# GadGadGad/Convolutional-KAN-for-Image-Classification

Hardware: AMD Instinct MI355X
Metric: images/sec fwd+bwd KAN-VGG11 3x32x32 bs=256/GPU (higher is better)
Workload: dtype f32

## Files before the change

### convolutional-kan-for-image-classification_amd/_lib.py

```python
from __future__ import annotations

import ctypes as C
import os
from typing import Optional

_HERE = os.path.dirname(os.path.abspath(__file__))
LIB_PATH = os.environ.get("KANCONV_LIB") or os.path.join(_HERE, "libkanconv.so")

KAN_MAX_PLANES = 16
KAN_MAX_TABLE = 32
KAN_FP_WORDS = 192
BASIS_BSPLINE, BASIS_RBF, BASIS_CHEBY, BASIS_POLY, BASIS_FOURIER, BASIS_RELU, BASIS_GRAM = 0, 1, 2, 3, 4, 5, 6
ACT_NONE, ACT_IDENTITY, ACT_GELU, ACT_SILU, ACT_RELU, ACT_TANH, ACT_SIGMOID, ACT_GELU_TANH = -1, 0, 1, 2, 3, 4, 5, 6
ORDER_QUAD_FWD, ORDER_ROWBLK8_FWD, ORDER_QUAD_BWD_DATA, ORDER_FWD_WEIGHT_SIDE = 1, 2, 4, 8


class KanGeom(C.Structure):
    _fields_ = [(n, C.c_int) for n in ("B", "C", "H", "W", "O", "Ho", "Wo", "kh", "kw", "sh", "sw", "ph", "pw", "dh", "dw", "groups")] + \
               [("x_bstride", C.c_longlong), ("y_bstride", C.c_longlong)]


class KanBasis(C.Structure):
    _fields_ = [("kind", C.c_int), ("n_basis", C.c_int), ("order", C.c_int), ("act", C.c_int),
                ("p0", C.c_float), ("p1", C.c_float), ("table", C.c_float * KAN_MAX_TABLE), ("chan_table", C.c_void_p)]


class KanPlan(C.Structure):
    _fields_ = [(n, C.c_int) for n in ("P", "K", "IPC", "KC", "Kpad", "Opad", "fwd_splits", "bwd_data_splits", "bwd_weight_splits",
                                          "fwd_target", "bwd_data_target", "bwd_weight_target", "x_pm_wanted", "dz_pm_wanted", "bwd_weight_expanded", "row_blocks", "e_pm_wanted", "fwd_expanded", "fwd_halo", "bwd_weight_halo",
                                          "fwd_band", "bwd_weight_band")] + \
               [(n, C.c_longlong) for n in ("packed_weight_bytes", "bwd_data_weight_bytes", "fwd_slab_elems", "bwd_data_slab_elems",
                                            "bwd_weight_slab_elems", "e_pm_elems")]


class KanNormRoute(C.Structure):
    _fields_ = [(n, C.c_int) for n in ("kernel", "G", "EPL", "PPI", "NT", "pool", "lds", "held", "blocks", "strided")]


NORM_GENERIC, NORM_REGS = 0, 1
NORM_POOL_NONE, NORM_POOL_2X2, NORM_POOL_K = 0, 1, 2


class KanWavGeom(C.Structure):
    _fields_ = [(n, C.c_int) for n in ("B", "C", "H", "W", "O", "Ho", "Wo", "kh", "kw", "sh", "sw", "ph", "pw", "dh", "dw", "wavelet")] + \
               [("x_bstride", C.c_longlong), ("u_bstride", C.c_longlong)]


# ... 113 lines not shown
```

### convolutional-kan-for-image-classification_amd/csrc/kan_common.h

```cpp
#pragma once
#include <hip/hip_runtime.h>
#include <cstdint>
#include <type_traits>
#include "kanconv.h"
#include "kan_device.h"
#include "kan_internal.h"

typedef float f32x16 __attribute__((ext_vector_type(16)));
#define MFMA32(a, b, c) __builtin_amdgcn_mfma_f32_32x32x2f32((a), (b), (c), 0, 0, 0)
#define LDS_READ4(r0, r1, r2, r3, addrA, addrB, o0, o1, o2, o3)                                                        \
    asm volatile("ds_read_b32 %0, %4 offset:%6\n\tds_read_b32 %1, %4 offset:%7\n\tds_read_b32 %2, %5 offset:%8\n\tds_read_b32 %3, %5 offset:%9" \
                 : "=&v"(r0), "=&v"(r1), "=&v"(r2), "=&v"(r3) : "v"(addrA), "v"(addrB), "n"(o0), "n"(o1), "n"(o2), "n"(o3) : "memory")
#define LDS_WAIT4(r0, r1, r2, r3, N) asm volatile("s_waitcnt lgkmcnt(" #N ")" : "+v"(r0), "+v"(r1), "+v"(r2), "+v"(r3) :: "memory")
__device__ __forceinline__ unsigned lds_addr(const float* p) { return (unsigned)(size_t)(__attribute__((address_space(3))) const float*)p; }
#define KAN_MFMA_STEP(NK, addrA, LDA, addrB, LDB)                                                                                   \
    do {                                                                                                                           \
        float fa_[2][2], fb_[2][2];                                                                                                \
        LDS_READ4(fa_[0][0], fa_[0][1], fb_[0][0], fb_[0][1], addrA, addrB, 0, 32 * 4, 0, 32 * 4);                                 \
        _Pragma("unroll") for (int kk = 0; kk < (NK); ++kk) {                                                                       \
            const int c_ = kk & 1, n_ = c_ ^ 1;                                                                                    \
            if (kk + 1 < (NK)) {                                                                                                   \
                LDS_READ4(fa_[n_][0], fa_[n_][1], fb_[n_][0], fb_[n_][1], addrA, addrB, (2 * (kk + 1)) * (LDA) * 4,                \
                          (2 * (kk + 1)) * (LDA) * 4 + 128, (2 * (kk + 1)) * (LDB) * 4, (2 * (kk + 1)) * (LDB) * 4 + 128);         \
                LDS_WAIT4(fa_[c_][0], fa_[c_][1], fb_[c_][0], fb_[c_][1], 4);                                                      \
            } else {                                                                                                               \
                LDS_WAIT4(fa_[c_][0], fa_[c_][1], fb_[c_][0], fb_[c_][1], 0);                                                      \
            }                                                                                                                      \
            acc[0][0] = MFMA32(fa_[c_][0], fb_[c_][0], acc[0][0]);                                                                 \
            acc[0][1] = MFMA32(fa_[c_][0], fb_[c_][1], acc[0][1]);                                                                 \
            acc[1][0] = MFMA32(fa_[c_][1], fb_[c_][0], acc[1][0]);                                                                 \
            acc[1][1] = MFMA32(fa_[c_][1], fb_[c_][1], acc[1][1]);                                                                 \
        }                                                                                                                          \
    } while (0)

#define KAN_MFMA_STEP_LIVE(NK, addrA, LDA, addrB, LDB, l0a, l0b, l1a, l1b)                                                          \
    do {                                                                                                                           \
        float fa_[2][2], fb_[2][2];                                                                                                \
        LDS_READ4(fa_[0][0], fa_[0][1], fb_[0][0], fb_[0][1], addrA, addrB, 0, 32 * 4, 0, 32 * 4);                                 \
        _Pragma("unroll") for (int kk = 0; kk < (NK); ++kk) {                                                                       \
            const int c_ = kk & 1, n_ = c_ ^ 1;                                                                                    \
            if (kk + 1 < (NK)) {                                                                                                   \
                LDS_READ4(fa_[n_][0], fa_[n_][1], fb_[n_][0], fb_[n_][1], addrA, addrB, (2 * (kk + 1)) * (LDA) * 4,                \
                          (2 * (kk + 1)) * (LDA) * 4 + 128, (2 * (kk + 1)) * (LDB) * 4, (2 * (kk + 1)) * (LDB) * 4 + 128);         \
                LDS_WAIT4(fa_[c_][0], fa_[c_][1], fb_[c_][0], fb_[c_][1], 4);                                                      \
            } else {                                                                                                               \
                LDS_WAIT4(fa_[c_][0], fa_[c_][1], fb_[c_][0], fb_[c_][1], 0);                                                      \
            }                                                                                                                      \
            if (kk < (NK) / 2 ? (l0a) : (l0b)) {                                                                                   \
                acc[0][0] = MFMA32(fa_[c_][0], fb_[c_][0], acc[0][0]);                                                             \
                acc[1][0] = MFMA32(fa_[c_][1], fb_[c_][0], acc[1][0]);                                                             \
            }                                                                                                                      \
            if (kk < (NK) / 2 ? (l1a) : (l1b)) {                                                                                   \
                acc[0][1] = MFMA32(fa_[c_][0], fb_[c_][1], acc[0][1]);                                                             \
                acc[1][1] = MFMA32(fa_[c_][1], fb_[c_][1], acc[1][1]);                                                             \
            }                                                                                                                      \
        }                                                                                                                          \
    } while (0)

namespace {

struct FastDiv { unsigned m; int s; };
__host__ __device__ inline FastDiv make_fastdiv(int d) {
    FastDiv f; f.s = 0;
    while ((1ll << f.s) < d) ++f.s;
    f.m = (unsigned)((((1ull << f.s) - (unsigned long long)d) << 32) / (unsigned long long)d + 1ull);
    return f;
}
__device__ __forceinline__ int fastdiv(int a, FastDiv f) {
    if (f.s == 0) return a;
    const unsigned t = __umulhi((unsigned)a, f.m);
    return (int)((t + (((unsigned)a - t) >> 1)) >> (f.s - 1));
}

template <int G>
__device__ __forceinline__ float group_sum(float v) {
#pragma unroll
    for (int off = G / 2; off >= 1; off >>= 1) v += __shfl_xor(v, off, 64);
    return v;
}
template <int G>
__device__ __forceinline__ double group_sum(double v) {
#pragma unroll
    for (int off = G / 2; off >= 1; off >>= 1) v += __shfl_xor(v, off, 64);
    return v;
}

struct DevGeom {
    int B, C, H, W, O, Ho, Wo, kh, kw, sh, sw, ph, pw, dh, dw;
    int howo_shift, wo_shift;
    int pix_major;
// ... 309 lines not shown
```

### convolutional-kan-for-image-classification_amd/csrc/kan_internal.h

```cpp
#pragma once
#include <type_traits>
#include "kanconv.h"

int kan_fail_msg(const char* fmt, const char* a);
int kan_raise_lds_limit(const void* kernel, int bytes);

enum : int {
    FAST_GENERIC = 0,
    FAST_BSPLINE_SILU = 1,
    FAST_BSPLINE_GELU = 2,
    FAST_RBF8 = 3,
    FAST_CHEBY5 = 4,
    FAST_CHEBY4 = 5,
    FAST_POLY4 = 6,
    FAST_POLY3 = 7,
    FAST_RBF5 = 8,
    FAST_RELU8 = 9,
    FAST_GRAM4 = 10,
    FAST_POLY1 = 11,
    FAST_LAST = 11
};
enum : unsigned {
    ON_TAP_MAJOR = 1u << 0,
    ON_BIG_TILES = 1u << 1,
// ... 75 lines not shown
    unsigned short bw_ph_rt0[KAN_BAND_MAX_PHASES + 1];
    unsigned char ph_a[KAN_BAND_MAX_PHASES], ph_b[KAN_BAND_MAX_PHASES];
    short ph_tap0[KAN_BAND_MAX_PHASES + 1];
    unsigned short tap_shift[KAN_BAND_MAX_TAPS];
    unsigned short tap_rt[KAN_BAND_MAX_TAPS];
    short tap_step[KAN_BAND_MAX_TAPS], tap_nt[KAN_BAND_MAX_TAPS];
} KanBandCfg;

void kan_band_cfg(const KanGeom* g, const KanBasis* b, int fast, KanBandCfg* cfg);
int kan_band_bwd_weight_launch(const float* dz, const float* x, const float* xn, float* dwp, const KanGeom* g, const KanBasis* b,
                               const KanBandCfg* cfg, int splits, long long slab_elems, void* stream);
int kan_band_fwd_launch(const float* x, const float* xn, const float* wp, float* z, const KanGeom* g, const KanBasis* b,
                        const KanBandCfg* cfg, int splits, long long slab_elems, void* stream);

constexpr int DW_T = 9;
constexpr int DW_MAX_TP = 96;

enum class Route { TAP_MAJOR, DW, BAND, HALO, EXPANDED };

struct FwdCfg { int TO, TP, tiles_o, tiles_p, chunks, splits, slots; };
struct BdCfg { int CH, tiles_c, tiles_p, n_ob, Opad32, chunks, splits; };
struct BwCfg { int TR, TO, tiles_r, tiles_o, chunks, splits, slots; };
struct BwHaloCfg { int R, nimg, spb, n_bands, tiles_r, tiles_o, splits, bands_per_split; };

struct ConvPlan {
    KanPlan pub;
    int fast;
    Route fwd, bwd_data, bwd_weight;
    bool pm_fwd, pm_bwd_data, pm_bwd_weight;
    bool rowblk_bwd_data;
    bool quad_fwd;
    bool quad_bd;
    bool rowblk8_fwd;
    bool fwd_wq;
    bool pmdma_xcd, pm_lpt, pm_xcd;
    FwdCfg fc;
    BdCfg bd;
    BwCfg bw;
    BwHaloCfg bwh;
    KanBandCfg band;
};
int plan_conv(const KanGeom* g, const KanBasis* b, ConvPlan* cp);

int live_taps_out(const KanGeom* g, int hw);
int live_taps_in(const KanGeom* g, int hw);
int live_positions_for_tap(const KanGeom* g, int tap);
int balance_tiles(const int* weight, int n, unsigned short* idx);
```

### convolutional-kan-for-image-classification_amd/csrc/kan_plan.hip

```cpp
#include <hip/hip_runtime.h>
#include <cstdio>
#include <cstdlib>
#include <cstring>
#include "kanconv.h"
#include "kan_device.h"
#include "kan_common.h"
#include "kan_internal.h"

namespace {

int fail(const char* msg) { return kan_fail_msg("%s", msg); }

int check(const KanGeom* g, const KanBasis* b) {
    if (!g || !b) return fail("null geometry/basis");
    if (g->groups < 0 || g->groups > 65535) return fail("groups out of range");
    if (g->B <= 0 || g->C <= 0 || g->O <= 0 || g->H <= 0 || g->W <= 0 || g->Ho <= 0 || g->Wo <= 0) return fail("non-positive dimension");
    if (g->kh <= 0 || g->kw <= 0 || g->sh <= 0 || g->sw <= 0 || g->dh <= 0 || g->dw <= 0 || g->ph < 0 || g->pw < 0) return fail("bad conv parameters");
    if (g->kh > 255 || g->kw > 255 || g->C > 65535) return fail("kernel size / channel count out of supported range");
    if ((g->H + 2 * g->ph - g->dh * (g->kh - 1) - 1) / g->sh + 1 != g->Ho || (g->W + 2 * g->pw - g->dw * (g->kw - 1) - 1) / g->sw + 1 != g->Wo)
        return fail("Ho/Wo inconsistent with H/W, kernel, stride, padding, dilation");
    if ((long long)g->B * g->Ho * g->Wo >= (1ll << 31) || (long long)g->B * g->H * g->W >= (1ll << 31)) return fail("pixel count exceeds int32");
    if ((long long)g->B * g->x_bstride * 4 >= (1ll << 31) || (long long)g->B * g->y_bstride * 4 >= (1ll << 31))
        return fail("activation tensors must be smaller than 2 GiB (32-bit buffer offsets)");
    if (g->x_bstride < (long long)ngroups(g) * g->C * g->H * g->W || g->y_bstride < (long long)ngroups(g) * g->O * g->Ho * g->Wo)
// ... 101 lines not shown
    if (g->kh != 3 || g->kw != 3 || g->sh != 1 || g->sw != 1 || g->dh != 1 || g->dw != 1 || g->ph != 1 || g->pw != 1) return false;
    if ((g->C & 1) || g->O % 128 != 0) return false;
    if (pm_fwd) return false;
    const int W = g->W, H = g->H;
    return (W == 32 && H % 4 == 0) || (W == 16 && H % 8 == 0) || (W == 8 && H == 8) || (W == 4 && H == 4);
}
bool band_fwd(const KanGeom* g, const KanBasis* b, int f, bool dw, bool pm_fwd, bool halo, KanBandCfg* out) {
    if (tuning_off("KAN_BAND") || !fast_has(f, ON_BAND_FWD)) return false;
    if (b->kind == KAN_BASIS_POLY && b->order == 0) return false;
    if (dw || pm_fwd || halo) return false;
    if (!(g->C <= 3 || round_up(g->O, 64) % 128 != 0 || (g->kh * g->kw >= 4 && g->C % 2 == 0 && !tuning_off("KAN_BAND_WIDE")))) return false;
    kan_band_cfg(g, b, f, out);
    return out->ok != 0;
}
FwdCfg fwd_cfg(const KanGeom* g, const KanPlan& pl, bool big, bool pm_fwd, bool halo) {
    FwdCfg c;
    c.TO = (big && !pm_fwd) ? 256 : (pl.Opad % 128 == 0) ? 128 : 64;
    c.slots = c.TO == 256 ? 512 : 1024;
    c.TP = 128;
    c.tiles_o = pl.Opad / c.TO;
    c.tiles_p = ceil_div((long long)g->B * g->Ho * g->Wo, c.TP);
    c.chunks = pl.Kpad / pl.KC;
    c.splits = pick_splits((long long)c.tiles_o * c.tiles_p * ngroups(g), c.chunks, 8, 4.0 * g->B * g->O * g->Ho * g->Wo * ngroups(g), c.slots);
    if (halo) {
        const int n_pairs = g->C / 2, pps = ceil_div(n_pairs, c.splits < n_pairs ? c.splits : n_pairs);
        c.splits = ceil_div(n_pairs, pps);
    }
    return c;
}
bool rowblk_bwd_data(const KanGeom* g, int f, bool pm_bwd_data) {
    return !tuning_off("KAN_BD_ROWBLK") && fast_has(f, ON_ROWBLK_BWD_DATA) && !pm_bwd_data && g->H == 4 && g->W == 4 && g->Ho == 4 && g->Wo == 4 &&
           g->kh == 3 && g->kw == 3 && g->sh == 1 && g->sw == 1 && g->ph == 1 && g->pw == 1 && g->dh == 1 && g->dw == 1 && g->B % 8 == 0 && g->O % 16 == 0;
}
struct LiveClass { long long tiles; int live_steps; };

int pick_target_steps(const LiveClass* cls, int ncls, int min_steps, double slab_bytes, int* max_splits, long long SLOTS = 1024) {
    int hi = 1;
    for (int i = 0; i < ncls; ++i) if (cls[i].live_steps > hi) hi = cls[i].live_steps;
    int best = hi; double best_cost = -1; int best_ms = 1;
    for (int t = min_steps < hi ? min_steps : hi; t <= hi; ++t) {
        long long wgs = 0; int ms = 1;
        for (int i = 0; i < ncls; ++i) {
            const int sp = cls[i].live_steps > 0 ? ceil_div(cls[i].live_steps, t) : 1;
            wgs += cls[i].tiles * sp;
            if (sp > ms) ms = sp;
        }
        const long long rounds = (wgs + SLOTS - 1) / SLOTS;
        const double cost = (double)(rounds * (t + 6)) + ms * slab_cost_steps(slab_bytes);
        if (best_cost < 0 || cost < best_cost) { best_cost = cost; best = t; best_ms = ms; }
    }
    *max_splits = best_ms;
    return best;
}
BdCfg bd_cfg(const KanGeom* g, const KanPlan& pl) {
    BdCfg c;
    c.CH = 64 / pl.P;
    c.tiles_c = ceil_div(g->C, 2 * c.CH);
    c.tiles_p = ceil_div((long long)g->B * g->H * g->W, 128);
    c.n_ob = ceil_div(g->O, 16);
    c.Opad32 = round_up(g->O, 32);
    c.chunks = g->kh * g->kw * c.n_ob;
    c.splits = pick_splits((long long)c.tiles_c * c.tiles_p * ngroups(g), c.chunks, 8, 4.0 * g->B * g->C * g->H * g->W * ngroups(g));
    return c;
}
bool pmdma_bwd_weight(const KanGeom* g, const KanBasis* b, int f, bool want_pm_bw) {
    if (tuning_off("KAN_PMDMA") || !fast_has(f, ON_EXPANDED)) return false;
// ... 98 lines not shown
        order[j] = v;
    }
    for (int r = 0; r < n; ++r) {
        const int depth = r / 8, k = r % 8, bin = (depth & 1) ? 7 - k : k;
        int slot = depth * 8 + bin;
        if (slot >= n) slot = r;
        idx[slot] = (unsigned short)order[r];
    }
    bool seen[PERM_MAX] = {false};
    for (int i = 0; i < n; ++i) { if (idx[i] >= n || seen[idx[i]]) return 0; seen[idx[i]] = true; }
    return n;
}

int plan_conv(const KanGeom* g, const KanBasis* b, ConvPlan* cp) {
    if (int rc = check(g, b)) return rc;
    ConvPlan& c = *cp;
    KanPlan* pl = &c.pub;
    const int T = g->kh * g->kw, G = ngroups(g), f = fast_variant(b);
    c.fast = f;
    const bool pm_shape = pmdma_fwd_shape(g, f);
    c.pm_fwd = want_pix_major(g, b, PM_FWD, pm_shape);
    c.pm_bwd_data = want_pix_major(g, b, PM_BWD_DATA, false);
    const bool want_pm_bw = want_pix_major(g, b, PM_BWD_WEIGHT, false);
    const bool dw = dw_direct(g, b);
    const bool halo = halo_fwd(g, b, f, c.pm_fwd);
    c.band.ok = c.band.bw_ok = 0;
    const bool band = band_fwd(g, b, f, dw, c.pm_fwd, halo, &c.band);
    const bool pmdma_fwd = pm_shape && c.pm_fwd;
    const bool pmdma_bw = pmdma_bwd_weight(g, b, f, want_pm_bw);
    const bool halo_bw = halo_bwd_weight(g, f, pmdma_bw);
    c.pm_bwd_weight = want_pm_bw && !halo_bw;
    const bool band_bw = band && c.band.bw_ok && !want_pm_bw && !tuning_off("KAN_BAND_BW");
    c.rowblk_bwd_data = rowblk_bwd_data(g, f, c.pm_bwd_data);
    c.pmdma_xcd = tuning_on("KAN_PMDMA_XCD");
    c.pm_lpt = !tuning_off("KAN_PM_LPT");
    c.pm_xcd = !tuning_off("KAN_PM_XCD");
    c.fwd = dw ? Route::DW : band ? Route::BAND : halo ? Route::HALO : pmdma_fwd ? Route::EXPANDED : Route::TAP_MAJOR;
    c.bwd_data = dw ? Route::DW : Route::TAP_MAJOR;
    c.bwd_weight = dw ? Route::DW : band_bw ? Route::BAND : halo_bw ? Route::HALO : pmdma_bw ? Route::EXPANDED : Route::TAP_MAJOR;
    pl->P = b->n_basis + (b->act != KAN_ACT_NONE);
    pl->K = g->C * T * pl->P;
    {
        int i18 = 18 / pl->P, i16 = 16 / pl->P;
        if (i18 > 4) i18 = 4;
        if (i16 > 4) i16 = 4;
        const bool use18 = (long long)i18 * pl->P * 16 > (long long)i16 * pl->P * 18;
        pl->KC = use18 ? 18 : 16;
        pl->IPC = use18 ? i18 : i16;
        if (pl->P >= 10 && pl->P <= 12) { pl->KC = 12; pl->IPC = 1; }
        if (halo) { pl->KC = 2 * pl->P; pl->IPC = 2; }
    }
    pl->Kpad = ceil_div(g->C * T, pl->IPC) * pl->KC;
    if (band) { pl->KC = c.band.NPLE; pl->IPC = c.band.NG; pl->Kpad = c.band.n_steps * c.band.NPLE; }
    pl->Opad = round_up(g->O, 64);
    pl->packed_weight_bytes = (long long)G * pl->Kpad * pl->Opad * 4;
    c.bd = bd_cfg(g, *pl);
    pl->bwd_data_weight_bytes = (long long)G * T * c.bd.Opad32 * c.bd.tiles_c * 128 * 4;
    pl->fwd_slab_elems = (long long)g->B * g->y_bstride;
    pl->bwd_data_slab_elems = (long long)g->B * g->x_bstride;
    pl->bwd_weight_slab_elems = (long long)G * pl->K * pl->Opad;
    const bool big = big_tiles(f, *pl);
    c.fc = fwd_cfg(g, *pl, big, c.pm_fwd, halo);
    c.bw = bw_cfg(g, *pl, big, c.pm_bwd_weight);
    if (halo_bw) c.bwh = bw_halo_cfg(g, *pl);
    pl->fwd_splits = band ? c.band.fwd_splits : c.fc.splits;
    pl->bwd_data_splits = c.bd.splits;
// ... 50 lines not shown
```

### convolutional-kan-for-image-classification_amd/csrc/kanconv.hip

```cpp
#include <hip/hip_runtime.h>
#include <cstdio>
#include <cstdlib>
#include <cstring>
#include <cmath>
#include <cstdint>
#include <mutex>
#include <type_traits>
#include <vector>
#include "kanconv.h"
#include "kan_device.h"

#include "kan_common.h"
#include "kan_internal.h"

namespace {


thread_local char g_err[512] = "";
int fail(const char* fmt, const char* a = "") {
    snprintf(g_err, sizeof(g_err), fmt, a);
    return -1;
}
}
int kan_fail_msg(const char* fmt, const char* a) { return fail(fmt, a); }
// ... 2731 lines not shown
    if (iod) {
        const IodLaunch l = iod_launch(g, pl);
        hipLaunchKernelGGL(k_pack_iod, dim3(l.blocks), dim3(256), 0, st, w_basis, wp, q, l.o_tiles, l.n_tiles, iod_vec(w_basis, wp, g, b));
    } else {
        hipLaunchKernelGGL(k_pack, grid, dim3(256), 0, st, w_base, w_basis, wp, q, nb_base, wp_gs, tiles_x, tiles_y, fp, fp_cur);
    }
    if (wd && cp.bwd_data == Route::DW) {
        if (hipMemcpyAsync(wd, wp, (size_t)pl.packed_weight_bytes, hipMemcpyDeviceToDevice, st) != hipSuccess) return fail("memcpy failed");
    } else if (wd) {
        const BdCfg& c = cp.bd;
        const int bx = c.tiles_c * 4, by = c.Opad32 / 32 * G;
        const long long nt = (long long)bx * by;
        const long long capd = fp ? 128 : 1024;
        dim3 gd((unsigned)(nt < capd ? nt : capd), 1, T);
        hipLaunchKernelGGL(k_pack_bwd_data, gd, dim3(256), 0, st, (const float*)wp, wd, q, c.CH, c.tiles_c, c.Opad32, wp_gs, bx, by, fp, fp_cur);
    }
    return launch_ok("pack");
}

int kan_pack_weights(const float* w_base, const float* w_basis, float* wp, float* wd, const KanGeom* g, const KanBasis* b, void* stream) {
    return pack_weights_impl(w_base, w_basis, wp, wd, g, b, nullptr, 0, stream);
}

int kan_pack_weights_iod(const float* coeffs, float* wp, float* wd, const KanGeom* g, const KanBasis* b, void* stream) {
    if (int rc = iod_scope(g, b)) return rc;
    return pack_weights_impl(nullptr, coeffs, wp, wd, g, b, nullptr, 0, stream, true);
}

int kan_tile_orders(const KanGeom* g, const KanBasis* b) {
    ConvPlan cp;
    if (plan_conv(g, b, &cp)) return 0;
    const bool halo = cp.fwd == Route::HALO;
    return (halo && cp.quad_fwd ? KAN_ORDER_QUAD_FWD : 0) | (halo && cp.rowblk8_fwd ? KAN_ORDER_ROWBLK8_FWD : 0) | (cp.quad_bd ? KAN_ORDER_QUAD_BWD_DATA : 0) |
           (cp.fwd_wq ? KAN_ORDER_FWD_WEIGHT_SIDE : 0);
}

int kan_pack_cacheable(const KanGeom* g, const KanBasis* b) {
    ConvPlan cp;
    if (plan_conv(g, b, &cp)) return 0;
    if ((long long)g->O * g->C * (b->n_basis + 1) * g->kh * g->kw >= (1ll << 31)) return 0;
    return (!pack_needs_clear(g, cp.pub) && cp.fwd != Route::DW && ngroups(g) == 1) ? 1 : 0;
}

int kan_pack_weights_cached(const float* w_base, const float* w_basis, float* wp, float* wd, const KanGeom* g, const KanBasis* b,
                            unsigned long long* ring, int cur, int force, int sample_stride, void* stream) {
    static_assert(KAN_FP_WORDS == 3 * FP_LANES, "ring size");
    if (!ring || cur < 0 || cur > 2 || sample_stride < 1) return fail("bad fingerprint ring arguments");
    if (!kan_pack_cacheable(g, b)) return fail("cached packing is not offered for this geometry (kan_pack_cacheable)");
    const int hb = b->act != KAN_ACT_NONE;
    if ((hb && !w_base) || !w_basis) return fail("null weight pointer");
    if (((size_t)w_basis & 15) || (hb && ((size_t)w_base & 15))) return fail("cached packing needs 16-byte aligned weight tensors");
    const int T = g->kh * g->kw;
    const long long na = hb ? (long long)g->O * g->C * T : 0, nbs = (long long)g->O * g->C * b->n_basis * T;
    const long long groups4 = ((na + 3) / 4 + (nbs + 3) / 4 + sample_stride - 1) / sample_stride;
    long long blocks = (groups4 + 256 * 8 - 1) / (256 * 8); if (blocks > 4096) blocks = 4096; if (blocks < 1) blocks = 1;
    hipLaunchKernelGGL(k_fingerprint, dim3((unsigned)blocks), dim3(256), 0, (hipStream_t)stream, hb ? w_base : w_basis, (unsigned)na, w_basis,
                       (unsigned)nbs, (unsigned)sample_stride, ring, cur);
    if (int rc = launch_ok("fingerprint")) return rc;
    return pack_weights_impl(w_base, w_basis, wp, wd, g, b, force ? nullptr : ring, cur, stream);
}

static int unpack_wgrad_impl(const float* dwp, float* dw_base, float* dw_basis, const KanGeom* g, const KanBasis* b, void* stream, bool iod) {
    ConvPlan cp;
    if (int rc = plan_conv(g, b, &cp)) return rc;
    const KanPlan& pl = cp.pub;
    const int hb = b->act != KAN_ACT_NONE;
    if ((hb && !dw_base) || !dw_basis || !dwp) return fail("null weight-gradient pointer");
// ... 152 lines not shown
    if ((b->kind == KAN_BASIS_RELU || b->kind == KAN_BASIS_GRAM) && !b->chan_table) return fail("ReLU / Gram bases need their device parameter table (chan_table)");
    if (!dxn && x != xn) return fail("dxn is required when xn != x");
    hipStream_t st = (hipStream_t)stream;
    if (cp.bwd_data == Route::DW) {
        DevGeom dgd = dev_geom(g); DevBasis dbd = dev_basis(b);
        dim3 grid(ceil_div((long long)g->B * g->H * g->W, 256), ngroups(g));
        dispatch_kind(b->kind, [&](auto kind) {
            hipLaunchKernelGGL((k_dw_bwd_data<decltype(kind)::value>), grid, dim3(256), 0, st, dz, x, xn, wd, dx, dxn, dgd, dbd, pl.Opad, pl.IPC, pl.KC, pl.Kpad);
        });
        return launch_ok("dw_bwd_data");
    }
    const BdCfg& c = cp.bd;
    DevGeom dg = dev_geom(g);
    dg.pix_major = (dz_pm && cp.pm_bwd_data) ? 1 : 0;
    if (dg.pix_major) dz = dz_pm;
    DevBasis db = dev_basis(b);
    if ((long long)c.tiles_c * ngroups(g) > 65535) return fail("groups * channel tiles exceed the grid limit");
    dim3 grid(c.tiles_p, c.tiles_c * ngroups(g), pl.bwd_data_splits);
    const int cps = dg.pix_major ? pl.bwd_data_target : ceil_div(c.chunks, pl.bwd_data_splits);
    TilePerm perm; perm.n = 0;
    if (dg.pix_major) perm = tile_perm(c.tiles_p, [&](int t) {
        const int hw = (int)(((long long)t * 128) / g->B);
        return ceil_div(live_taps_in(g, hw < g->H * g->W ? hw : 0) * c.n_ob, cps > 0 ? cps : 1);
    });
    const int fast = (fast_spec(cp.fast).xn_bwd ? (x != xn && dxn) : (x == xn && !dxn)) ? cp.fast : FAST_GENERIC;
    const bool rb = !dg.pix_major && cp.rowblk_bwd_data;
    const bool quad = rb && cp.quad_bd && dz_pm && x == xn && !dxn;
    const unsigned dz_bytes = (unsigned)((long long)g->B * g->y_bstride * 4);
    auto launch = [&](auto kind, auto fast, auto rbv) {
        hipLaunchKernelGGL((k_conv_bwd_data<decltype(kind)::value, decltype(fast)::value, decltype(rbv)::value>), grid, dim3(256), 0, st,
                           decltype(rbv)::value == 2 ? dz_pm : dz, x, xn, wd,
                           dx, dxn, dg, db, c.CH, c.tiles_c, c.n_ob, c.Opad32, c.chunks, cps, pl.bwd_data_slab_elems, dz_bytes, perm, dpar);
    };
    const bool launched = dispatch_fast<ON_TAP_MAJOR>(fast, [&](auto fv) {
        constexpr int F = decltype(fv)::value;
        if constexpr (fast_has(F, ON_ROWBLK_BWD_DATA)) {
            if (quad) return launch(IC<fast_kind(F)>{}, fv, IC<2>{});
            if (rb) return launch(IC<fast_kind(F)>{}, fv, IC<1>{});
        }
        launch(IC<fast_kind(F)>{}, fv, IC<0>{});
    });
    if (!launched) dispatch_kind(b->kind, [&](auto kind) { launch(kind, IC<FAST_GENERIC>{}, IC<0>{}); });
    return launch_ok("conv_bwd_data");
}

int kan_conv_bwd_weight(const float* dz, const float* x, const float* xn, float* dwp, const KanGeom* g, const KanBasis* b,
                        const float* x_pm, const float* dz_pm, void* stream) {
    ConvPlan cp;
    if (int rc = plan_conv(g, b, &cp)) return rc;
    const KanPlan& pl = cp.pub;
    if (!dz || !x || !xn || !dwp) return fail("null tensor pointer");
    if ((b->kind == KAN_BASIS_RELU || b->kind == KAN_BASIS_GRAM) && !b->chan_table) return fail("ReLU / Gram bases need their device parameter table (chan_table)");
    hipStream_t st = (hipStream_t)stream;
    if (cp.bwd_weight == Route::DW) {
        DevGeom dgd = dev_geom(g); DevBasis dbd = dev_basis(b);
        dim3 grid(pl.bwd_weight_splits, ngroups(g));
        dispatch_kind(b->kind, [&](auto kind) {
            hipLaunchKernelGGL((k_dw_bwd_weight<decltype(kind)::value>), grid, dim3(256), 0, st, dz, x, xn, dwp, dgd, dbd, pl.K, pl.Opad, pl.bwd_weight_slab_elems);
        });
        return launch_ok("dw_bwd_weight");
    }
    if (cp.bwd_weight == Route::BAND) {
        if (x != xn && !fast_spec(cp.fast).xn_fwd) return fail("this basis / activation pair runs on single-input kernels: pass xn == x");
        return kan_band_bwd_weight_launch(dz, x, xn, dwp, g, b, &cp.band, pl.bwd_weight_splits, pl.bwd_weight_slab_elems, stream);
    }
    const unsigned x_bytes = (unsigned)((long long)g->B * g->x_bstride * 4), dz_bytes = (unsigned)((long long)g->B * g->y_bstride * 4);
// ... 374 lines not shown
```

### convolutional-kan-for-image-classification_amd/ops.py

```python
from __future__ import annotations

import contextlib
import ctypes as C
import os
import weakref
from collections import OrderedDict
from dataclasses import dataclass, replace
from functools import lru_cache, partial, wraps
from typing import List, NamedTuple, Optional, Sequence, Tuple

import torch
from torch.autograd.function import once_differentiable

from . import _lib as L


@dataclass(frozen=True)
class ConvSpec:
    kind: int
    n_basis: int
    order: int
    act: int
    p0: float
    p1: float
# ... 147 lines not shown


def _conv_flops(geom, plan) -> float:
    return 2.0 * geom.B * geom.O * geom.Ho * geom.Wo * geom.C * plan.P * geom.kh * geom.kw * max(1, geom.groups)


@lru_cache(maxsize=256)
def _live_fraction(which: str, H: int, W: int, Ho: int, Wo: int, kh: int, kw: int, sh: int, sw: int, ph: int, pw: int, dh: int, dw: int) -> float:
    live = 0
    for ho in range(Ho):
        for wo in range(Wo):
            for r in range(kh):
                for t in range(kw):
                    hi, wi = ho * sh - ph + r * dh, wo * sw - pw + t * dw
                    live += 0 <= hi < H and 0 <= wi < W
    return live / float(Ho * Wo * kh * kw)


_ROW_BLOCK_BIT = {"fwd": 1, "bwd_data": 2, "bwd_weight": 0}


def _quadrant_order(geom, plan, which: str) -> bool:
    return which == "fwd" and bool(plan.row_blocks & 1) and geom.B % 32 == 0


def _quadrant_bwd_data(geom, plan, have_dz_pm: bool) -> bool:
    return bool(have_dz_pm) and bool(plan.row_blocks & 2) and bool(getattr(plan, "tile_orders", 0) & L.ORDER_QUAD_BWD_DATA)


def _row_blocks8_forward(geom, plan) -> bool:
    return geom.H == 8 and geom.W == 8 and bool(getattr(plan, "tile_orders", 0) & L.ORDER_ROWBLK8_FWD)


def _executed_flops(geom, plan, which: str, have_dz_pm: bool = False) -> float:
    target = {"fwd": plan.fwd_target, "bwd_data": plan.bwd_data_target, "bwd_weight": plan.bwd_weight_target}[which]
    dense = _conv_flops(geom, plan)
    g = geom
    if target <= 0:
        if _quadrant_order(geom, plan, which) or (which == "bwd_data" and _quadrant_bwd_data(geom, plan, have_dz_pm)):
            return dense * _live_fraction(which, g.H, g.W, g.Ho, g.Wo, g.kh, g.kw, g.sh, g.sw, g.ph, g.pw, g.dh, g.dw)
        if plan.row_blocks & _ROW_BLOCK_BIT[which]:
            return dense * (5.0 / 6.0)
        if which == "fwd" and _row_blocks8_forward(geom, plan):
            return dense * (11.0 / 12.0)
        return dense
    return dense * _live_fraction(which, g.H, g.W, g.Ho, g.Wo, g.kh, g.kw, g.sh, g.sw, g.ph, g.pw, g.dh, g.dw)


def _layer_tag(geom) -> str:
    return f"{geom.C * max(1, geom.groups)}->{geom.O * max(1, geom.groups)}@{geom.H}x{geom.W} k{geom.kh}x{geom.kw}"


def _sample(which: str, geom, plan, pm: bool, two: bool = False, expanded: bool = False):
    tile = "128" if plan.Opad % 128 == 0 else "64"
    if which == "bwd_data":
        name = "k_conv_bwd_data"
    elif expanded:
        name = f"k_conv_{which}_pmdma/o{tile}"
    elif plan.fwd_band if which == "fwd" else plan.bwd_weight_band:
        name = f"k_band_{which}/o" + ("128" if plan.Opad % 128 == 0 else "192" if plan.Opad == 192 else "64")
    else:
        halo = plan.fwd_halo if which == "fwd" else (plan.bwd_weight_halo and not two)
        name = f"k_conv_{which}{'_halo' if halo else ''}/o{tile}"
    skips = expanded or pm or bool(plan.row_blocks & _ROW_BLOCK_BIT[which]) or (which == "fwd" and _row_blocks8_forward(geom, plan))
    dense = _conv_flops(geom, plan)
    return name, dense, _executed_flops(geom, plan, which, pm) if skips else dense, _layer_tag(geom)


def _position_major(t: torch.Tensor, ch_off: int, Cn: int) -> torch.Tensor:
    B, Ct, H, W = t.shape
    out = torch.empty(Cn * H * W * B, device=t.device, dtype=torch.float32)
    L.check(L.load().kan_position_major(_ptr(t, ch_off * H * W), _ptr(out), B, Cn, H * W, Ct * H * W, _stream(t)), "kan_position_major")
    return out


def _stack(ws: Sequence[Optional[torch.Tensor]]) -> Optional[torch.Tensor]:
    if ws[0] is None:
        return None
    return ws[0].unsqueeze(0) if len(ws) == 1 else torch.stack(list(ws))


_PACKED: "OrderedDict[tuple, PackedWeights]" = OrderedDict()
_PACK_CACHE_MAX = int(os.environ.get("KAN_PACK_CACHE", "256"))
_PACK_CACHE_BYTES = int(os.environ.get("KAN_PACK_CACHE_BYTES", str(16 << 30)))
_PACK_SAMPLE = max(1, int(os.environ.get("KAN_PACK_SAMPLE", "1")))
_PACK_VERIFY_EVERY = int(os.environ.get("KAN_PACK_VERIFY_EVERY", "16"))
_EPOCH = 0
PACK_STATS = {"calls": 0, "forced": 0, "skipped": 0}


_ALWAYS_PACK = False


@contextlib.contextmanager
def always_pack():
    global _ALWAYS_PACK
# ... 380 lines not shown
    elif exact_w:
        dwp = torch.empty(plan.bwd_weight_splits * plan.bwd_weight_slab_elems, device=x.device, dtype=torch.float32)
        if plan.bwd_weight_expanded and xn is None and dz_pm is not None:
            e_pm = x_pm if (plan.fwd_expanded and not plan.x_pm_wanted and x_pm is not None and mode == 0) else _expand_pm(x, geom, basis, plan, st)
            _launch(_sample("bwd_weight", geom, plan, True, expanded=True), x,
                    lambda: lib.kan_conv_bwd_weight_expanded(_ptr(dz_pm), _ptr(e_pm), _ptr(dwp), C.byref(geom), C.byref(basis), st))
        else:
            _launch(_sample("bwd_weight", geom, plan, x_pm is not None and dz_pm is not None, xn is not None), x,
                    lambda: lib.kan_conv_bwd_weight(_ptr(dz), _ptr(x), _ptr(xs), _ptr(dwp), C.byref(geom), C.byref(basis), _ptr(x_pm),
                                                    _ptr(dz_pm), st))
        if spec.w_layout == W_IOD:
            dco = torch.empty((Cg, Og, spec.n_basis), device=x.device, dtype=torch.float32)
            L.check(lib.kan_unpack_wgrad_iod(_ptr(dwp), _ptr(dco), C.byref(geom), C.byref(basis), st), "kan_unpack_wgrad_iod")
            dw_basis = [dco]
        else:
            sb = _sink_for(wids[0], (Og, Cg, kh, kw), x.device) if (wids and G == 1 and spec.has_base) else None
            ss = _sink_for(wids[1], (Og, Cg * spec.n_basis, kh, kw), x.device) if (wids and G == 1) else None
            dwb = (sb.unsqueeze(0) if sb is not None else
                   torch.empty((G, Og, Cg, kh, kw), device=x.device, dtype=torch.float32)) if spec.has_base else None
            dws = ss.unsqueeze(0) if ss is not None else torch.empty((G, Og, Cg * spec.n_basis, kh, kw), device=x.device, dtype=torch.float32)
            L.check(lib.kan_unpack_wgrad(_ptr(dwp), _ptr(dwb), _ptr(dws), C.byref(geom), C.byref(basis), st), "kan_unpack_wgrad")
            dw_basis = list(dws.unbind(0))
            if spec.has_base:
                dw_base = list(dwb.unbind(0))
    dx = dxn = None
    if split_x:
        dx, _ = kan_conv_bwd_data_split(spec, x, dz, None, None, wcd)
    elif exact_x:
        S = plan.bwd_data_splits
        separate = xn is not None
        dxs = torch.empty((S, B, Ct, H, W), device=x.device, dtype=torch.float32)
        dxns = torch.empty_like(dxs) if separate else None
        head, tail = (_ptr(dz), _ptr(x), _ptr(xs), _ptr(wd), _ptr(dxs), _ptr(dxns)), (C.byref(geom), C.byref(basis), _ptr(dz_pm), st)
        _launch(_sample("bwd_data", geom, plan, dz_pm is not None), x,
                (lambda: lib.kan_conv_bwd_data(*head, *tail)) if dparams is None else
                (lambda: lib.kan_conv_bwd_data_params(*head, _ptr(dparams), *tail)))
        dx, dxn = _sum_slabs(dxs, B, Ct, H * W), (_sum_slabs(dxns, B, Ct, H * W) if separate else None)
    return dx, dxn, dw_base, dw_basis


def _sum_slabs(slabs: torch.Tensor, B: int, Cn: int, HW: int) -> torch.Tensor:
    if slabs.shape[0] == 1:
        return slabs[0]
    out = torch.empty_like(slabs[0])
    L.check(L.load().kan_slab_reduce(_ptr(slabs), slabs.shape[0], slabs[0].numel(), _ptr(out), B, Cn, HW, Cn * HW, _stream(slabs)),
            "kan_slab_reduce")
    return out


def _flat_grads(spec: ConvSpec, dw_base, dw_basis):
    return tuple(dw_base) + tuple(dw_basis) if spec.has_base else tuple(dw_basis)


def _save(ctx, **named) -> None:
    ctx.saved_names = tuple(k for k, t in named.items() if t is not None)
    ctx.save_for_backward(*(t for t in named.values() if t is not None))


def _once(backward):
    inner = once_differentiable(backward)

    @wraps(backward)
    def wrapper(ctx, *grads):
        if torch.is_grad_enabled() and not any(g is not None and g.requires_grad for g in grads):
            grads = tuple(g.detach().requires_grad_(True) if g is not None else None for g in grads)
        return inner(ctx, *grads)
    return wrapper
# ... 545 lines not shown
```

### include/kanconv.h

```cpp
#ifndef KANCONV_H
#define KANCONV_H

#ifdef __cplusplus
extern "C" {
#endif

#define KAN_MAX_PLANES 16
#define KAN_MAX_TABLE  32
#define KAN_FP_WORDS   192

enum { KAN_BASIS_BSPLINE = 0, KAN_BASIS_RBF = 1, KAN_BASIS_CHEBY = 2, KAN_BASIS_POLY = 3, KAN_BASIS_FOURIER = 4, KAN_BASIS_RELU = 5, KAN_BASIS_GRAM = 6 };
enum { KAN_ACT_NONE = -1, KAN_ACT_IDENTITY = 0, KAN_ACT_GELU = 1, KAN_ACT_SILU = 2, KAN_ACT_RELU = 3,
       KAN_ACT_TANH = 4, KAN_ACT_SIGMOID = 5, KAN_ACT_GELU_TANH = 6 };

typedef struct KanGeom {
    int B, C, H, W;
    int O, Ho, Wo;
    int kh, kw, sh, sw, ph, pw, dh, dw;
    int groups;
    long long x_bstride;
    long long y_bstride;
} KanGeom;

#define KAN_ORDER_PACK(mode, first) ((int)(mode) | ((int)(first) << 8))
// ... 5 lines not shown
    float table[KAN_MAX_TABLE];
    const float* chan_table;
} KanBasis;

typedef struct KanPlan {
    int P;
    int K;
    int IPC, KC;
    int Kpad, Opad;
    int fwd_splits;
    int bwd_data_splits;
    int bwd_weight_splits;
    int fwd_target, bwd_data_target, bwd_weight_target;
    int x_pm_wanted, dz_pm_wanted;
    int bwd_weight_expanded;
    int row_blocks;
    int e_pm_wanted, fwd_expanded;
    int fwd_halo, bwd_weight_halo;
    int fwd_band, bwd_weight_band;
    long long packed_weight_bytes;
    long long bwd_data_weight_bytes;
    long long fwd_slab_elems;
    long long bwd_data_slab_elems;
    long long bwd_weight_slab_elems;
    long long e_pm_elems;
} KanPlan;

const char* kan_version(void);
const char* kan_last_error(void);

int kan_plan(const KanGeom* geom, const KanBasis* basis, KanPlan* plan);

#define KAN_ORDER_QUAD_FWD 1
#define KAN_ORDER_ROWBLK8_FWD 2
#define KAN_ORDER_QUAD_BWD_DATA 4
#define KAN_ORDER_FWD_WEIGHT_SIDE 8
int kan_tile_orders(const KanGeom* geom, const KanBasis* basis);

int kan_pack_weights(const float* w_base, const float* w_basis, float* wp, float* wd,
                     const KanGeom* geom, const KanBasis* basis, void* stream);

int kan_pack_weights_iod(const float* coeffs, float* wp, float* wd, const KanGeom* geom, const KanBasis* basis, void* stream);

int kan_pack_cacheable(const KanGeom* geom, const KanBasis* basis);
int kan_pack_weights_cached(const float* w_base, const float* w_basis, float* wp, float* wd,
                            const KanGeom* geom, const KanBasis* basis, unsigned long long* ring, int cur, int force,
                            int sample_stride, void* stream);

int kan_conv_fwd(const float* x, const float* xn, const float* wp, float* z,
                 const KanGeom* geom, const KanBasis* basis, const float* x_pm, void* stream);

int kan_position_major(const float* src, float* dst, int B, int Cn, int HW, long long bstride, void* stream);

int kan_conv_bwd_data(const float* dz, const float* x, const float* xn, const float* wd,
                      float* dx, float* dxn,
                      const KanGeom* geom, const KanBasis* basis, const float* dz_pm, void* stream);

int kan_conv_bwd_data_params(const float* dz, const float* x, const float* xn, const float* wd, float* dx, float* dxn, float* dparams,
                             const KanGeom* geom, const KanBasis* basis, const float* dz_pm, void* stream);

int kan_conv_bwd_weight(const float* dz, const float* x, const float* xn, float* dwp,
                        const KanGeom* geom, const KanBasis* basis, const float* x_pm, const float* dz_pm, void* stream);

int kan_position_major_expanded(const float* x, float* e_pm, const KanGeom* geom, const KanBasis* basis, void* stream);
int kan_conv_fwd_expanded(const float* e_pm, const float* wp, float* z, const KanGeom* geom, const KanBasis* basis, void* stream);
int kan_conv_fwd_expanded_order(const float* e_pm, const float* wp, float* z, const KanGeom* geom, const KanBasis* basis, void* stream, int order);
// ... 151 lines not shown
```

Measured before the change: 18170.

## Add 8x8 row-block bwd-data MFMA kernel for 3x3 stride-1 layers

```diff
diff --git a/convolutional-kan-for-image-classification_amd/_lib.py b/convolutional-kan-for-image-classification_amd/_lib.py
--- a/convolutional-kan-for-image-classification_amd/_lib.py
+++ b/convolutional-kan-for-image-classification_amd/_lib.py
@@ -12,7 +12,7 @@
 KAN_FP_WORDS = 192
 BASIS_BSPLINE, BASIS_RBF, BASIS_CHEBY, BASIS_POLY, BASIS_FOURIER, BASIS_RELU, BASIS_GRAM = 0, 1, 2, 3, 4, 5, 6
 ACT_NONE, ACT_IDENTITY, ACT_GELU, ACT_SILU, ACT_RELU, ACT_TANH, ACT_SIGMOID, ACT_GELU_TANH = -1, 0, 1, 2, 3, 4, 5, 6
-ORDER_QUAD_FWD, ORDER_ROWBLK8_FWD, ORDER_QUAD_BWD_DATA, ORDER_FWD_WEIGHT_SIDE = 1, 2, 4, 8
+ORDER_QUAD_FWD, ORDER_ROWBLK8_FWD, ORDER_QUAD_BWD_DATA, ORDER_FWD_WEIGHT_SIDE, ORDER_ROWBLK8_BWD_DATA = 1, 2, 4, 8, 16
 
 
 class KanGeom(C.Structure):
diff --git a/convolutional-kan-for-image-classification_amd/csrc/kan_bwd8.hip b/convolutional-kan-for-image-classification_amd/csrc/kan_bwd8.hip
--- /dev/null
+++ b/convolutional-kan-for-image-classification_amd/csrc/kan_bwd8.hip
@@ -0,0 +1,160 @@
+#include <hip/hip_runtime.h>
+#include <cstdint>
+#include "kanconv.h"
+#include "kan_device.h"
+#include "kan_common.h"
+#include "kan_internal.h"
+
+namespace {
+
+template <int KIND, int FAST>
+__global__ __launch_bounds__(512, 2) void k_conv_bwd_data_rb8(
+    const float* __restrict__ dz, const float* __restrict__ x, const float* __restrict__ wd, float* __restrict__ dx, DevGeom g, DevBasis bs,
+    int n_ct, int n_ob, int Opad16, int n_chunks, int chunks_per_split, long long slab_elems, unsigned dz_bytes) {
+    constexpr FastSpec S = fast_spec(FAST);
+    static_assert(FAST != 0 && !S.xn_bwd, "single-tensor compile-time specs only");
+    constexpr int IMS = 72, LDG = 4 * IMS, KD = 16, FP = S.planes, FCH = 64 / FP, NIT = (FCH + 3) / 4;
+    constexpr int BUF = KD * 128 + KD * LDG;
+    __shared__ __attribute__((aligned(16))) float smem[2 * BUF];
+    __shared__ float sTab[KAN_MAX_TABLE];
+
+    const int tid = threadIdx.x, lane = tid & 63;
+    const int wave = __builtin_amdgcn_readfirstlane(tid >> 6);
+    const int ws = wave & 3, w_r = ws >> 1, w_p = (wave >> 2) ? ((ws & 1) ? 2 : 1) : ((ws & 1) ? 3 : 0);
+    const BlockId blk = xcd_block_order(false);
+    const int grp = blk.y / n_ct, ct = blk.y - grp * n_ct;
+    const int img0 = blk.x * 4, ncol = n_ct * 128;
+    const bool idle_rows = (ct * 2 + w_r) * FCH >= g.C;
+    {
+        const size_t xo = (size_t)grp * g.C * 64;
+        x += xo; dx += xo;
+        dz += (size_t)grp * g.O * 64;
+        wd += (size_t)grp * 9 * Opad16 * ncol;
+    }
+    if (tid < KAN_MAX_TABLE) sTab[tid] = bs.tab[tid];
+
+    const int g_row = lane >> 3, g_w = lane & 7, ol0 = wave >> 2;
+    const kan_rsrc dz_rs = make_rsrc(dz, dz_bytes);
+    const unsigned dz_img = (unsigned)(img0 + ws) * (unsigned)g.ybs;
+    const unsigned wlane = (unsigned)((lane >> 5) * ncol + (lane & 31) * 4) * 4u;
+    constexpr unsigned row_bytes = 64u * 4u;
+
+    int rb_t = -1; unsigned baseA = KAN_OOB, baseB = KAN_OOB; bool pend_mixed = false;
+    auto issue = [&](int ch, int buf) {
+        const int n_plain = 3 * n_ob;
+        const bool mixed = ch >= n_plain;
+        pend_mixed = mixed;
+        int t, o0;
+        if (mixed) { const int m = ch - n_plain; t = m / (2 * n_ob); o0 = (m - t * 2 * n_ob) * 8; }
+        else { t = ch / n_ob; o0 = (ch - t * n_ob) * KD; }
+        const int key = mixed ? 3 + t : t;
+        if (key != rb_t) {
+            rb_t = key;
+            const int wn = g_w + 1 - t;
+            const bool okw = wn >= 0 && wn < 8;
+            const int hA = g_row + 1 - (mixed ? 0 : 1), hB = g_row + 1 - 2;
+            baseA = (okw && hA >= 0 && hA < 8) ? (dz_img + (unsigned)(hA * 8 + wn)) * 4u : KAN_OOB;
+            baseB = (okw && hB >= 0 && hB < 8) ? (dz_img + (unsigned)(hB * 8 + wn)) * 4u : KAN_OOB;
+        }
+        float* dW = smem + buf * BUF;
+        float* dG = dW + KD * 128 + ws * IMS;
+        const unsigned soA = (unsigned)(o0 + ol0) * row_bytes;
+        if (mixed) {
+#pragma unroll
+            for (int n = 0; n < 8; ++n)
+                __builtin_amdgcn_raw_ptr_buffer_load_lds(dz_rs, (__attribute__((address_space(3))) void*)(dG + (ol0 + 2 * n) * LDG), 4,
+                                                         (int)(n < 4 ? baseA : baseB), (int)(soA + (unsigned)(2 * (n & 3)) * row_bytes), 0, 0);
+        } else {
+#pragma unroll
+            for (int n = 0; n < 8; ++n)
+                __builtin_amdgcn_raw_ptr_buffer_load_lds(dz_rs, (__attribute__((address_space(3))) void*)(dG + (ol0 + 2 * n) * LDG), 4,
+                                                         (int)baseA, (int)(soA + (unsigned)(2 * n) * row_bytes), 0, 0);
+        }
+        const int tapA = mixed ? t : 3 + t, tapB = 6 + t;
+        const int row = mixed ? ((wave < 4 ? tapA : tapB) * Opad16 + o0 + ws * 2) : (tapA * Opad16 + o0 + wave * 2);
+        glds16((const float*)((const char*)(wd + (size_t)row * ncol + ct * 128) + wlane), dW + wave * 256);
+    };
+
+    f32x16 acc[2][2];
+#pragma unroll
+    for (int a = 0; a < 2; ++a)
+#pragma unroll
+        for (int b = 0; b < 2; ++b)
+#pragma unroll
+            for (int r = 0; r < 16; ++r) acc[a][b][r] = 0.f;
+
+    const int ch0 = blk.z * chunks_per_split, ch1 = min(n_chunks, ch0 + chunks_per_split);
+    int ch = ch0;
+    if (ch < ch1) issue(ch, 0);
+    const int ar = w_r * 64 + (lane & 31), bp = ((lane & 31) >> 3) * IMS + w_p * 16 + (lane & 7), kh2 = lane >> 5;
+    for (int cur = 0; ch < ch1; cur ^= 1) {
+        asm volatile("s_waitcnt vmcnt(0)" ::: "memory");
+        __syncthreads();
+        const bool mixed_now = pend_mixed;
+        ++ch;
+        const float* cW = smem + cur * BUF;
+        const float* cG = cW + KD * 128;
+        const unsigned aw = lds_addr(cW + kh2 * 128 + ar), ag = lds_addr(cG + kh2 * LDG + bp);
+        const bool l0b = !(mixed_now && w_p == 0), l1a = !(mixed_now && w_p == 3);
+        if (!idle_rows) KAN_MFMA_STEP_LIVE_B(KD / 2, aw, 128, ag, LDG, 8 * 4, true, l0b, l1a, true, if (ch < ch1) issue(ch, cur ^ 1));
+        else if (ch < ch1) issue(ch, cur ^ 1);
+    }
+
+    float* dxs = dx + (size_t)blk.z * slab_elems;
+    const int e_px = tid & 127, e_c0 = tid >> 7;
+    const int e_col = ((e_px >> 3) & 3) * 32 + (e_px >> 5) * 8 + (e_px & 7);
+    const size_t e_off = (size_t)(img0 + (e_px >> 5)) * g.xbs + (size_t)(e_px & 31);
+    float xv[4][NIT];
+#pragma unroll
+    for (int pass = 0; pass < 4; ++pass)
+#pragma unroll
+        for (int it = 0; it < NIT; ++it) {
+            const int cl = e_c0 + 4 * it, c = (ct * 2 + (pass >> 1)) * FCH + cl;
+            xv[pass][it] = (cl < FCH && c < g.C) ? x[e_off + (size_t)c * 64 + (size_t)((pass & 1) * 32)] : 0.f;
+        }
+#pragma unroll
+    for (int pass = 0; pass < 4; ++pass) {
+        const int half = pass >> 1, q = pass & 1;
+        __syncthreads();
+        if (w_r == half && (w_p >> 1) == q) {
+#pragma unroll
+            for (int mi = 0; mi < 2; ++mi)
+#pragma unroll
+                for (int ni = 0; ni < 2; ++ni)
+#pragma unroll
+                    for (int r = 0; r < 16; ++r)
+                        smem[(mi * 32 + mfma_row(r, lane)) * 128 + (w_p & 1) * 64 + ni * 32 + (lane & 31)] = acc[mi][ni][r];
+        }
+        __syncthreads();
+#pragma unroll
+        for (int it = 0; it < NIT; ++it) {
+            const int cl = e_c0 + 4 * it, c = (ct * 2 + half) * FCH + cl;
+            if (!(cl < FCH && c < g.C)) continue;
+            const InGrad d = stage_unit_grad<KIND, FAST>(bs, sTab, xv[pass][it], xv[pass][it], smem + (cl * FP) * 128 + e_col, 128);
+            dxs[e_off + (size_t)c * 64 + (size_t)(q * 32)] = d.dx;
+        }
+    }
+}
+
+}
+
+int kan_bwd_data_rb8_launch(const float* dz, const float* x, const float* wd, float* dx, const KanGeom* g, const KanBasis* b, const ConvPlan* cp,
+                            void* stream) {
+    const BdCfg& c = cp->bd;
+    const KanPlan& pl = cp->pub;
+    const DevGeom dg = dev_geom(g);
+    const DevBasis db = dev_basis(b);
+    const dim3 grid(g->B / 4, c.tiles_c * ngroups(g), pl.bwd_data_splits);
+    const int cps = ceil_div(c.chunks, pl.bwd_data_splits);
+    const unsigned dz_bytes = (unsigned)((long long)g->B * g->y_bstride * 4);
+    const bool launched = dispatch_fast<ON_TAP_MAJOR | ON_ROWBLK_BWD_DATA>(cp->fast, [&](auto fv) {
+        constexpr int F = decltype(fv)::value;
+        if constexpr (!fast_spec(F).xn_bwd)
+            hipLaunchKernelGGL((k_conv_bwd_data_rb8<fast_kind(F), F>), grid, dim3(512), 0, (hipStream_t)stream, dz, x, wd, dx, dg, db, c.tiles_c, c.n_ob,
+                               c.Opad32, c.chunks, cps, pl.bwd_data_slab_elems, dz_bytes);
+    });
+    if (!launched) return kan_fail_msg("internal: no 8x8 row-block bwd-data kernel for this basis%s", "");
+    const hipError_t e = hipGetLastError();
+    if (e != hipSuccess) { kan_fail_msg("launch failed: %s", hipGetErrorString(e)); return -2; }
+    return 0;
+}
diff --git a/convolutional-kan-for-image-classification_amd/csrc/kan_common.h b/convolutional-kan-for-image-classification_amd/csrc/kan_common.h
--- a/convolutional-kan-for-image-classification_amd/csrc/kan_common.h
+++ b/convolutional-kan-for-image-classification_amd/csrc/kan_common.h
@@ -33,15 +33,15 @@
         }                                                                                                                          \
     } while (0)
 
-#define KAN_MFMA_STEP_LIVE(NK, addrA, LDA, addrB, LDB, l0a, l0b, l1a, l1b)                                                          \
+#define KAN_MFMA_STEP_LIVE_B(NK, addrA, LDA, addrB, LDB, BOFF, l0a, l0b, l1a, l1b, MID)                                             \
     do {                                                                                                                           \
         float fa_[2][2], fb_[2][2];                                                                                                \
-        LDS_READ4(fa_[0][0], fa_[0][1], fb_[0][0], fb_[0][1], addrA, addrB, 0, 32 * 4, 0, 32 * 4);                                 \
+        LDS_READ4(fa_[0][0], fa_[0][1], fb_[0][0], fb_[0][1], addrA, addrB, 0, 32 * 4, 0, (BOFF));                                 \
         _Pragma("unroll") for (int kk = 0; kk < (NK); ++kk) {                                                                       \
             const int c_ = kk & 1, n_ = c_ ^ 1;                                                                                    \
             if (kk + 1 < (NK)) {                                                                                                   \
                 LDS_READ4(fa_[n_][0], fa_[n_][1], fb_[n_][0], fb_[n_][1], addrA, addrB, (2 * (kk + 1)) * (LDA) * 4,                \
-                          (2 * (kk + 1)) * (LDA) * 4 + 128, (2 * (kk + 1)) * (LDB) * 4, (2 * (kk + 1)) * (LDB) * 4 + 128);         \
+                          (2 * (kk + 1)) * (LDA) * 4 + 128, (2 * (kk + 1)) * (LDB) * 4, (2 * (kk + 1)) * (LDB) * 4 + (BOFF));      \
                 LDS_WAIT4(fa_[c_][0], fa_[c_][1], fb_[c_][0], fb_[c_][1], 4);                                                      \
             } else {                                                                                                               \
                 LDS_WAIT4(fa_[c_][0], fa_[c_][1], fb_[c_][0], fb_[c_][1], 0);                                                      \
@@ -54,8 +54,11 @@
                 acc[0][1] = MFMA32(fa_[c_][0], fb_[c_][1], acc[0][1]);                                                             \
                 acc[1][1] = MFMA32(fa_[c_][1], fb_[c_][1], acc[1][1]);                                                             \
             }                                                                                                                      \
+            if (kk == 0) { MID; }                                                                                                  \
         }                                                                                                                          \
     } while (0)
+
+#define KAN_MFMA_STEP_LIVE(NK, addrA, LDA, addrB, LDB, l0a, l0b, l1a, l1b) KAN_MFMA_STEP_LIVE_B(NK, addrA, LDA, addrB, LDB, 32 * 4, l0a, l0b, l1a, l1b, (void)0)
 
 namespace {
 
diff --git a/convolutional-kan-for-image-classification_amd/csrc/kan_internal.h b/convolutional-kan-for-image-classification_amd/csrc/kan_internal.h
--- a/convolutional-kan-for-image-classification_amd/csrc/kan_internal.h
+++ b/convolutional-kan-for-image-classification_amd/csrc/kan_internal.h
@@ -131,6 +131,7 @@
     bool quad_fwd;
     bool quad_bd;
     bool rowblk8_fwd;
+    bool rowblk8_bd;
     bool fwd_wq;
     bool pmdma_xcd, pm_lpt, pm_xcd;
     FwdCfg fc;
@@ -141,6 +142,9 @@
 };
 int plan_conv(const KanGeom* g, const KanBasis* b, ConvPlan* cp);
 
+int kan_bwd_data_rb8_launch(const float* dz, const float* x, const float* wd, float* dx, const KanGeom* g, const KanBasis* b, const ConvPlan* cp,
+                            void* stream);
+
 int live_taps_out(const KanGeom* g, int hw);
 int live_taps_in(const KanGeom* g, int hw);
 int live_positions_for_tap(const KanGeom* g, int tap);
diff --git a/convolutional-kan-for-image-classification_amd/csrc/kan_plan.hip b/convolutional-kan-for-image-classification_amd/csrc/kan_plan.hip
--- a/convolutional-kan-for-image-classification_amd/csrc/kan_plan.hip
+++ b/convolutional-kan-for-image-classification_amd/csrc/kan_plan.hip
@@ -157,6 +157,11 @@
     return !tuning_off("KAN_BD_ROWBLK") && fast_has(f, ON_ROWBLK_BWD_DATA) && !pm_bwd_data && g->H == 4 && g->W == 4 && g->Ho == 4 && g->Wo == 4 &&
            g->kh == 3 && g->kw == 3 && g->sh == 1 && g->sw == 1 && g->ph == 1 && g->pw == 1 && g->dh == 1 && g->dw == 1 && g->B % 8 == 0 && g->O % 16 == 0;
 }
+bool rowblk8_bwd_data(const KanGeom* g, int f, bool pm_bwd_data, bool dw) {
+    return !tuning_off("KAN_ROWBLK8_BD") && fast_has(f, ON_ROWBLK_BWD_DATA) && !fast_spec(f).xn_bwd && !pm_bwd_data && !dw && g->H == 8 && g->W == 8 &&
+           g->Ho == 8 && g->Wo == 8 && g->kh == 3 && g->kw == 3 && g->sh == 1 && g->sw == 1 && g->ph == 1 && g->pw == 1 && g->dh == 1 && g->dw == 1 &&
+           g->B % 4 == 0 && g->O % 16 == 0;
+}
 struct LiveClass { long long tiles; int live_steps; };
 
 int pick_target_steps(const LiveClass* cls, int ncls, int min_steps, double slab_bytes, int* max_splits, long long SLOTS = 1024) {
@@ -321,6 +326,7 @@
     c.pm_bwd_weight = want_pm_bw && !halo_bw;
     const bool band_bw = band && c.band.bw_ok && !want_pm_bw && !tuning_off("KAN_BAND_BW");
     c.rowblk_bwd_data = rowblk_bwd_data(g, f, c.pm_bwd_data);
+    c.rowblk8_bd = rowblk8_bwd_data(g, f, c.pm_bwd_data, dw);
     c.pmdma_xcd = tuning_on("KAN_PMDMA_XCD");
     c.pm_lpt = !tuning_off("KAN_PM_LPT");
     c.pm_xcd = !tuning_off("KAN_PM_XCD");
diff --git a/convolutional-kan-for-image-classification_amd/csrc/kanconv.hip b/convolutional-kan-for-image-classification_amd/csrc/kanconv.hip
--- a/convolutional-kan-for-image-classification_amd/csrc/kanconv.hip
+++ b/convolutional-kan-for-image-classification_amd/csrc/kanconv.hip
@@ -2787,7 +2787,7 @@
     if (plan_conv(g, b, &cp)) return 0;
     const bool halo = cp.fwd == Route::HALO;
     return (halo && cp.quad_fwd ? KAN_ORDER_QUAD_FWD : 0) | (halo && cp.rowblk8_fwd ? KAN_ORDER_ROWBLK8_FWD : 0) | (cp.quad_bd ? KAN_ORDER_QUAD_BWD_DATA : 0) |
-           (cp.fwd_wq ? KAN_ORDER_FWD_WEIGHT_SIDE : 0);
+           (cp.fwd_wq ? KAN_ORDER_FWD_WEIGHT_SIDE : 0) | (cp.rowblk8_bd ? KAN_ORDER_ROWBLK8_BWD_DATA : 0);
 }
 
 int kan_pack_cacheable(const KanGeom* g, const KanBasis* b) {
@@ -3006,6 +3006,8 @@
                            decltype(rbv)::value == 2 ? dz_pm : dz, x, xn, wd,
                            dx, dxn, dg, db, c.CH, c.tiles_c, c.n_ob, c.Opad32, c.chunks, cps, pl.bwd_data_slab_elems, dz_bytes, perm, dpar);
     };
+    const bool rb8 = !dg.pix_major && cp.rowblk8_bd && x == xn && !dxn && !dpar;
+    if (rb8) return kan_bwd_data_rb8_launch(dz, x, wd, dx, g, b, &cp, stream);
     const bool launched = dispatch_fast<ON_TAP_MAJOR>(fast, [&](auto fv) {
         constexpr int F = decltype(fv)::value;
         if constexpr (fast_has(F, ON_ROWBLK_BWD_DATA)) {
diff --git a/convolutional-kan-for-image-classification_amd/ops.py b/convolutional-kan-for-image-classification_amd/ops.py
--- a/convolutional-kan-for-image-classification_amd/ops.py
+++ b/convolutional-kan-for-image-classification_amd/ops.py
@@ -203,6 +203,10 @@
     return geom.H == 8 and geom.W == 8 and bool(getattr(plan, "tile_orders", 0) & L.ORDER_ROWBLK8_FWD)
 
 
+def _row_blocks8_bwd_data(plan) -> bool:
+    return bool(getattr(plan, "tile_orders", 0) & L.ORDER_ROWBLK8_BWD_DATA)
+
+
 def _executed_flops(geom, plan, which: str, have_dz_pm: bool = False) -> float:
     target = {"fwd": plan.fwd_target, "bwd_data": plan.bwd_data_target, "bwd_weight": plan.bwd_weight_target}[which]
     dense = _conv_flops(geom, plan)
@@ -233,6 +237,9 @@
     else:
         halo = plan.fwd_halo if which == "fwd" else (plan.bwd_weight_halo and not two)
         name = f"k_conv_{which}{'_halo' if halo else ''}/o{tile}"
+    if which == "bwd_data" and not two and _row_blocks8_bwd_data(plan):
+        dense = _conv_flops(geom, plan)
+        return name, dense, dense * (11.0 / 12.0), _layer_tag(geom)
     skips = expanded or pm or bool(plan.row_blocks & _ROW_BLOCK_BIT[which]) or (which == "fwd" and _row_blocks8_forward(geom, plan))
     dense = _conv_flops(geom, plan)
     return name, dense, _executed_flops(geom, plan, which, pm) if skips else dense, _layer_tag(geom)
@@ -679,7 +686,7 @@
         dxs = torch.empty((S, B, Ct, H, W), device=x.device, dtype=torch.float32)
         dxns = torch.empty_like(dxs) if separate else None
         head, tail = (_ptr(dz), _ptr(x), _ptr(xs), _ptr(wd), _ptr(dxs), _ptr(dxns)), (C.byref(geom), C.byref(basis), _ptr(dz_pm), st)
-        _launch(_sample("bwd_data", geom, plan, dz_pm is not None), x,
+        _launch(_sample("bwd_data", geom, plan, dz_pm is not None, xn is not None or dparams is not None), x,
                 (lambda: lib.kan_conv_bwd_data(*head, *tail)) if dparams is None else
                 (lambda: lib.kan_conv_bwd_data_params(*head, _ptr(dparams), *tail)))
         dx, dxn = _sum_slabs(dxs, B, Ct, H * W), (_sum_slabs(dxns, B, Ct, H * W) if separate else None)
diff --git a/include/kanconv.h b/include/kanconv.h
--- a/include/kanconv.h
+++ b/include/kanconv.h
@@ -61,6 +61,7 @@
 int kan_plan(const KanGeom* geom, const KanBasis* basis, KanPlan* plan);
 
 #define KAN_ORDER_QUAD_FWD 1
+#define KAN_ORDER_ROWBLK8_BWD_DATA 16
 #define KAN_ORDER_ROWBLK8_FWD 2
 #define KAN_ORDER_QUAD_BWD_DATA 4
 #define KAN_ORDER_FWD_WEIGHT_SIDE 8
```

New measurement: 18230 (median of 6 runs). No clear change (+0.4%).
